# ALVI-Labs/frankenstein

Hardware: AMD Instinct MI355X
Metric: neural frames/sec (train fwd+bwd+AdamW, whole job) (higher is better)
Workload: dtype bf16; 1 GPU; brainformer-small (6L d=384 6x64 heads, N=6144 tokens) + 2-block perceiver, L1 head; fwd+bwd+clip+AdamW; per_gpu_batch=32, global_batch=32, frames_T=600, electrodes=256, parallelism=dp1, weights=random-init (seed 42)

## Files before the change

### frankenstein_amd/csrc/mlp_fused.hip

```cpp
#include "fk_common.h"

namespace {

#include "gemm_tile.h"

typedef __attribute__((address_space(3))) void lds_void_t;
typedef __attribute__((address_space(1))) const void glb_void_t;
extern __shared__ __attribute__((aligned(16))) char smem[];

struct MlpBwdArgs {
  const bf16_t* dy; const bf16_t* w2t; const bf16_t* h13; const bf16_t* w13t;
  bf16_t* dh13; bf16_t* dx;
  int64_t lddy, ldw2t, ldh, ldw13t, lddh, lddx;
  int M, H;
};

constexpr int MF_D = 384, MF_NW = 4, MF_TOK = MF_NW * 32;
constexpr int MF_KT = MF_D / 64;
constexpr int MF_NT = MF_D / 32;
constexpr int MF_W2 = MF_KT * 32 * ROW_BYTES;
constexpr int MF_W13 = MF_D * ROW_BYTES;
constexpr int MF_SLOT = MF_W2 + MF_W13;
constexpr int MF_HREG = 32 * ROW_BYTES;
constexpr int MF_LDS = 2 * MF_SLOT + MF_NW * MF_HREG;
constexpr int MF_P2 = MF_W2 / 1024 / MF_NW;
constexpr int MF_P13 = MF_W13 / 1024 / MF_NW;
constexpr int MF_ROWP = MF_D * 2 + 16;
static_assert(MF_LDS <= 160 * 1024 && MF_TOK * MF_ROWP <= MF_LDS, "LDS of a CU");
static_assert(MF_SLOT % (1024 * MF_NW) == 0, "whole pieces per wave");

template <bool FAST_SIGMOID> FK_DEV float mf_sigmoid(float x) {
  if constexpr (FAST_SIGMOID) return __builtin_amdgcn_rcpf(1.0f + __expf(-x));
  else return 1.0f / (1.0f + __expf(-x));
}

FK_DEV void mf_dma(const void* base, unsigned voff, unsigned dst) {
  asm volatile("s_mov_b32 m0, %2\n\ts_nop 0\n\tglobal_load_lds_dwordx4 %0, %1" ::"v"(voff), "s"(base), "s"(dst) : "memory");
}
FK_DEV void wait_all_barrier() { asm volatile("s_waitcnt vmcnt(0)\n\ts_barrier" ::: "memory"); }

struct LaneIds {
  int lane, li, lh, wave, row8, ch;
  FK_DEV LaneIds() {
    const int tid = threadIdx.x;
    lane = tid & 63, li = lane & 31, lh = lane >> 5;
    wave = __builtin_amdgcn_readfirstlane(tid >> 6);
    row8 = lane >> 3, ch = lane & 7;
  }
};
FK_DEV int swz_col(int r, int ch) { return (ch ^ ((r >> 1) & 7)) << 3; }
FK_DEV unsigned row_byte_off(int row, int64_t ld, int col) { return (unsigned)(((int64_t)row * ld + col) * 2); }

FK_DEV void load_token_frags(Frag<bf16_t> (&f)[MF_D / 16], const bf16_t* base, int row, int64_t ld, int lh) {
  const bf16_t* src = base + (int64_t)row * ld + 8 * lh;
#pragma unroll
  for (int t = 0; t < MF_D / 16; ++t) frag_load_contig<bf16_t>(f[t], src + 16 * t);
}
template <int N> FK_DEV void zero_acc(f32x16 (&a)[N]) {
#pragma unroll
  for (int t = 0; t < N; ++t)
#pragma unroll
    for (int r = 0; r < 16; ++r) a[t][r] = 0.0f;
}

template <int N> FK_DEV void row_segments(bf16_t* (&dst)[N], bool (&ok)[N], bf16_t* base, int64_t ld, int row0, int step, int M, int col) {
#pragma unroll
  for (int j = 0; j < N; ++j) {
    const int mr = row0 + j * step;
    ok[j] = mr < M;
    dst[j] = base + (int64_t)(ok[j] ? mr : M - 1) * ld + col;
  }
}
FK_DEV void read_tile_rows(bf16x8 (&rb)[4], const char* tile, const LaneIds& L) {
#pragma unroll
  for (int j = 0; j < 4; ++j) rb[j] = *reinterpret_cast<const bf16x8*>(tile + nt_off(j * 8 + L.row8, L.ch));
}
template <int N, bool NT> FK_DEV void store_rows(bf16_t* const (&dst)[N], const bool (&ok)[N], bool wave_full, int col, const bf16x8 (&v)[N]) {
  if (wave_full) {
#pragma unroll
    for (int j = 0; j < N; ++j) fk_st<NT>(reinterpret_cast<bf16x8*>(dst[j] + col), v[j]);
  } else {
#pragma unroll
    for (int j = 0; j < N; ++j)
      if (ok[j]) fk_st<NT>(reinterpret_cast<bf16x8*>(dst[j] + col), v[j]);
  }
}

struct BwdRing {
  const MlpBwdArgs& p;
  const LaneIds& L;
  unsigned lds0, off2[MF_P2], off13[MF_P13];
  FK_DEV BwdRing(const MlpBwdArgs& p_, const LaneIds& L_) : p(p_), L(L_), lds0((unsigned)(uintptr_t)(lds_void_t*)smem) {
#pragma unroll
    for (int j = 0; j < MF_P2; ++j) {
      const int q = L.wave * MF_P2 + j, s6 = q >> 2, r = (q & 3) * 8 + L.row8;
      off2[j] = (unsigned)((r * (int)p.ldw2t + s6 * 64 + swz_col(r, L.ch)) * 2);
    }
#pragma unroll
    for (int j = 0; j < MF_P13; ++j) {
      const int r = (L.wave * MF_P13 + j) * 8 + L.row8;
      off13[j] = (unsigned)((r * (int)p.ldw13t + swz_col(r, L.ch)) * 2);
    }
  }
  template <typename B> static FK_DEV B w2_at(B base, int slot) { return base + slot * MF_W2; }
  template <typename B> static FK_DEV B w13_at(B base, int slot) { return base + 2 * MF_W2 + slot * MF_W13; }
  template <typename B> FK_DEV B tile_at(B base) const { return base + 2 * MF_SLOT + L.wave * MF_HREG; }
  FK_DEV const char* w2img(int slot) const { return w2_at(smem, slot); }
  FK_DEV const char* w13img(int slot) const { return w13_at(smem, slot); }
  FK_DEV char* tile() const { return tile_at(smem); }
  FK_DEV unsigned tile_lds() const { return __builtin_amdgcn_readfirstlane(tile_at(lds0)); }
  FK_DEV const bf16_t* w2_src(int c) const { return p.w2t + (int64_t)c * 32 * p.ldw2t; }
  FK_DEV const bf16_t* w13_src(int c) const { return p.w13t + (int64_t)c * 64; }
  FK_DEV const bf16_t* h_src(int c) const { return p.h13 + (int64_t)c * 64; }
  FK_DEV unsigned w2_dst(int slot) const { return __builtin_amdgcn_readfirstlane(w2_at(lds0, slot) + L.wave * (MF_W2 / MF_NW)); }
  FK_DEV unsigned w13_dst(int slot) const { return __builtin_amdgcn_readfirstlane(w13_at(lds0, slot) + L.wave * (MF_W13 / MF_NW)); }
  FK_DEV void dma_w2(int c, int slot, int j) const { mf_dma(w2_src(c), off2[j], w2_dst(slot) + j * 1024); }
  FK_DEV void dma_w13(int c, int slot, int j) const { mf_dma(w13_src(c), off13[j], w13_dst(slot) + j * 1024); }
  FK_DEV unsigned h_off(int j, int row) const { return row_byte_off(row, p.ldh, swz_col(j * 8 + L.row8, L.ch)); }
  FK_DEV void dma_h(int c, int j, unsigned hoff, unsigned tile_dst) const { mf_dma(h_src(c), hoff, tile_dst + j * 1024); }
  FK_DEV void issue_w2(int c, int slot) const {
#pragma unroll
    for (int j = 0; j < MF_P2; ++j) dma_w2(c, slot, j);
  }
  FK_DEV void issue_w13(int c, int slot) const {
#pragma unroll
    for (int j = 0; j < MF_P13; ++j) dma_w13(c, slot, j);
  }
  FK_DEV void issue_h(int c, const unsigned (&hoff)[4], unsigned tile_dst) const {
#pragma unroll
    for (int j = 0; j < 4; ++j) dma_h(c, j, hoff[j], tile_dst);
  }
};

template <typename F>
FK_DEV void first_product(f32x16& dg, Frag<bf16_t> (&fa)[2][4], const char* w2img, const Frag<bf16_t> (&dyf)[MF_D / 16], const LaneIds& L, const F& behind) {
#pragma unroll
  for (int r = 0; r < 16; ++r) dg[r] = 0.0f;
#pragma unroll
  for (int s = 0; s < 4; ++s) nt_frag<bf16_t>(fa[0][s], w2img, L.li, s, L.lh);
#pragma unroll
  for (int s6 = 0; s6 < MF_KT; ++s6) {
    if (s6 + 1 < MF_KT) {
#pragma unroll
      for (int s = 0; s < 4; ++s) nt_frag<bf16_t>(fa[(s6 + 1) & 1][s], w2img + (s6 + 1) * 32 * ROW_BYTES, L.li, s, L.lh);
    }
#pragma unroll
    for (int s = 0; s < 4; ++s) mma32<bf16_t>(dg, fa[s6 & 1][s], dyf[s6 * 4 + s]);
    behind(s6);
    __builtin_amdgcn_sched_group_barrier(0x100, 4, 0);
    __builtin_amdgcn_sched_group_barrier(0x008, 4, 0);
    __builtin_amdgcn_sched_barrier(0);
  }
}

FK_DEV bf16x8 dswiglu_piece(const bf16x8& hv, const f32x16& dg, int s) {
  bf16x8 o;
#pragma unroll
  for (int e = 0; e < 4; ++e) {
    const float a1 = (float)hv[e], a3 = (float)hv[4 + e], g = dg[4 * s + e];
    const float sg = mf_sigmoid<true>(a1), ds = g * sg;
    o[e] = (bf16_t)(ds * a3 * (1.0f + a1 * (1.0f - sg)));
    o[4 + e] = (bf16_t)(ds * a1);
  }
  return o;
}

template <typename F>
FK_DEV void second_product(f32x16 (&dx)[MF_NT], Frag<bf16_t> (&fa)[2][4], const char* w13img, const Frag<bf16_t> (&bf)[4], const LaneIds& L, const F& behind) {
#pragma unroll
  for (int s = 0; s < 4; ++s) nt_frag<bf16_t>(fa[0][s], w13img, L.li, s, L.lh);
#pragma unroll
  for (int t = 0; t < MF_NT; ++t) {
    if (t + 1 < MF_NT) {
#pragma unroll
      for (int s = 0; s < 4; ++s) nt_frag<bf16_t>(fa[(t + 1) & 1][s], w13img, 32 * (t + 1) + L.li, s, L.lh);
    }
#pragma unroll
    for (int s = 0; s < 4; ++s) mma32<bf16_t>(dx[t], fa[t & 1][s], bf[s]);
    behind(t);
    __builtin_amdgcn_sched_group_barrier(0x100, 4, 0);
    __builtin_amdgcn_sched_group_barrier(0x008, 4, 0);
    __builtin_amdgcn_sched_barrier(0);
  }
}

FK_DEV void store_dx(const MlpBwdArgs& p, const f32x16 (&dx)[MF_NT], const LaneIds& L, int m0w, int row_end) {
  char* stg = smem + L.wave * 32 * MF_ROWP;
#pragma unroll
  for (int t = 0; t < MF_NT; ++t)
#pragma unroll
    for (int g = 0; g < 4; ++g) {
      bf16x4 v;
#pragma unroll
      for (int e = 0; e < 4; ++e) v[e] = (bf16_t)dx[t][4 * g + e];
      *reinterpret_cast<bf16x4*>(stg + L.li * MF_ROWP + (32 * t + 8 * g + 4 * L.lh) * 2) = v;
    }
  asm volatile("s_waitcnt lgkmcnt(0)" ::: "memory");
  if (L.lane < MF_D / 8) {
    for (int r = 0; r < 32; ++r) {
      if (m0w + r >= row_end) break;
      const bf16x8 v = *reinterpret_cast<const bf16x8*>(stg + r * MF_ROWP + L.lane * 16);
      fk_st<true>(reinterpret_cast<bf16x8*>(p.dx + (int64_t)(m0w + r) * p.lddx + L.lane * 8), v);
    }
  }
}

#ifdef MF_STAMP
__device__ unsigned long long mf_stamp_acc[16];
#define MF_ST_DECL unsigned long long st_acc[10] = {0, 0, 0, 0, 0, 0, 0, 0, 0, 0}; unsigned long long st_t = __builtin_amdgcn_s_memtime(); const unsigned long long st_t0 = st_t;
#define MF_ST(i) { const unsigned long long t_ = __builtin_amdgcn_s_memtime(); st_acc[i] += t_ - st_t; st_t = t_; }
#define MF_ST_FLUSH(lane) if ((lane) == 0) { for (int i_ = 0; i_ < 10; ++i_) atomicAdd(&mf_stamp_acc[i_], st_acc[i_]); atomicAdd(&mf_stamp_acc[15], __builtin_amdgcn_s_memtime() - st_t0); }
#else
#define MF_ST_DECL
#define MF_ST(i)
#define MF_ST_FLUSH(lane)
#endif

__global__ __launch_bounds__(MF_NW * 64, 1) void mlp_bwd_fused_kernel(MlpBwdArgs p) {
  using T = bf16_t;
  const LaneIds L;
  const BwdRing ring(p, L);
  const int m0w = blockIdx.x * MF_TOK + L.wave * 32, m = m0w + L.li;
  const int mc = m < p.M ? m : p.M - 1;
  const bool wave_full = m0w + 32 <= p.M;
  const int nchunks = p.H / 32, last = nchunks - 1;
  char* hreg = ring.tile();
  const unsigned hreg_lds = ring.tile_lds();
  T* hdst[4];
  bool hrow_ok[4];
  row_segments(hdst, hrow_ok, p.dh13, p.lddh, m0w + L.row8, 8, p.M, L.ch << 3);
  unsigned hoff[4];
#pragma unroll
  for (int j = 0; j < 4; ++j) hoff[j] = ring.h_off(j, hrow_ok[j] ? m0w + j * 8 + L.row8 : p.M - 1);

  ring.issue_w2(0, 0);
  ring.issue_w13(0, 0);
  ring.issue_w2(last < 1 ? last : 1, 1);
  ring.issue_h(0, hoff, hreg_lds);
  Frag<T> dyf[MF_D / 16];
  load_token_frags(dyf, p.dy, mc, p.lddy, L.lh);
  f32x16 dx[MF_NT];
  zero_acc(dx);
  wait_all_barrier();

  for (int c = 0; c < nchunks; ++c) {
    if (c > 0) asm volatile("s_waitcnt vmcnt(26)\n\ts_barrier" ::: "memory");
    const int cn1 = c + 1 < nchunks ? c + 1 : last, cn2 = c + 2 < nchunks ? c + 2 : last;
    f32x16 dg;
    Frag<T> fa[2][4];
    first_product(dg, fa, ring.w2img(c & 1), dyf, L, [&](int s6) __attribute__((always_inline)) {
      ring.dma_w13(cn1, (c + 1) & 1, 2 * s6);
      ring.dma_w13(cn1, (c + 1) & 1, 2 * s6 + 1);
    });
    asm volatile("s_waitcnt vmcnt(12)" ::: "memory");
    Frag<T> bf[4];
#pragma unroll
    for (int s = 0; s < 4; ++s) {
      bf[s].v = dswiglu_piece(*reinterpret_cast<const bf16x8*>(hreg + nt_off(L.li, 2 * s + L.lh)), dg, s);
      *reinterpret_cast<bf16x8*>(hreg + nt_off(L.li, 2 * s + L.lh)) = bf[s].v;
    }
    bf16x8 rb[4];
    read_tile_rows(rb, hreg, L);
    asm volatile("s_waitcnt vmcnt(22)\n\ts_barrier" ::: "memory");
    store_rows<4, true>(hdst, hrow_ok, wave_full, c * 64, rb);
    second_product(dx, fa, ring.w13img(c & 1), bf, L, [&](int t) __attribute__((always_inline)) {
      if (t < MF_P2) ring.dma_w2(cn2, c & 1, t);
      else if (t < MF_P2 + 4) ring.dma_h(cn1, t - MF_P2, hoff[t - MF_P2], hreg_lds);
    });
  }
  wait_all_barrier();
  store_dx(p, dx, L, m0w, p.M);
}


typedef unsigned u32x16 __attribute__((ext_vector_type(16)));
typedef unsigned u32x4v __attribute__((ext_vector_type(4)));
#ifndef FK_MLPB_INC
#define FK_MLPB_INC "mlp_bwd_asm.inc"
#endif
#include FK_MLPB_INC

__global__ __launch_bounds__(MF_NW * 64, 1) void mlp_bwd_fused_asm_kernel(MlpBwdArgs p) {
  MF_ST_DECL
  using T = bf16_t;
  const LaneIds L;
  const BwdRing ring(p, L);
  const int m0w = blockIdx.x * MF_TOK + L.wave * 32;
  const int nchunks = p.H / 32, last = nchunks - 1;
  auto cl = [&](int k) { return k < last ? k : last; };
  char* hreg = ring.tile();
  const unsigned hreg_lds = ring.tile_lds();
  u32x16 adr, ofs;
  unsigned ax[4], hoff[4];
#pragma unroll
  for (int s = 0; s < 4; ++s) {
    ax[s] = (unsigned)nt_off(L.li, 2 * s + L.lh);
    adr[4 + s] = hreg_lds + ax[s];
    adr[8 + s] = hreg_lds + (unsigned)nt_off(s * 8 + L.row8, L.ch);
  }
#pragma unroll
  for (int j = 0; j < MF_P2; ++j) ofs[j] = ring.off2[j];
#pragma unroll
  for (int j = 0; j < 4; ++j) {
    hoff[j] = ring.h_off(j, m0w + j * 8 + L.row8);
    ofs[6 + j] = hoff[j];
    ofs[10 + j] = row_byte_off(m0w + j * 8 + L.row8, p.lddh, L.ch << 3);
  }
  ofs[14] = 0;
  ofs[15] = 0;

  ring.issue_w2(0, 0);
  ring.issue_w13(0, 0);
  ring.issue_w2(cl(1), 1);
  ring.issue_h(0, hoff, hreg_lds);
  Frag<T> dyf[MF_D / 16];
  load_token_frags(dyf, p.dy, m0w + L.li, p.lddy, L.lh);
  f32x16 dx[MF_NT];
  zero_acc(dx);
  MF_ST(4)
  wait_all_barrier();
  MF_ST(5)
  Frag<T> fa[2][4];
  f32x16 dg;
  u32x16 fa0, bfc, bfn, hvv;
  first_product(dg, fa, ring.w2img(0), dyf, L, [](int) {});
  {
    bf16x8 rb[4];
#pragma unroll
    for (int s = 0; s < 4; ++s) {
      const bf16x8 o = dswiglu_piece(*reinterpret_cast<const bf16x8*>(hreg + nt_off(L.li, 2 * s + L.lh)), dg, s);
      *reinterpret_cast<bf16x8*>(hreg + nt_off(L.li, 2 * s + L.lh)) = o;
      const u32x4v w = __builtin_bit_cast(u32x4v, o);
#pragma unroll
      for (int k = 0; k < 4; ++k) bfc[4 * s + k] = w[k];
    }
    read_tile_rows(rb, hreg, L);
#pragma unroll
    for (int j = 0; j < 4; ++j)
      fk_st<true>(reinterpret_cast<bf16x8*>(p.dh13 + (int64_t)(m0w + j * 8 + L.row8) * p.lddh + (L.ch << 3)), rb[j]);
  }
  asm volatile("s_waitcnt lgkmcnt(0)\n\ts_barrier" ::: "memory");
  ring.issue_w2(cl(2), 0);
  ring.issue_h(cl(1), hoff, hreg_lds);
#pragma unroll
  for (int s = 0; s < 4; ++s) {
    const u32x4v w = *reinterpret_cast<const u32x4v*>(ring.w2img(1) + ax[s]);
#pragma unroll
    for (int k = 0; k < 4; ++k) fa0[4 * s + k] = w[k];
  }

  MF_ST(0)
  for (int c = 0; c < last; ++c) {
    const char* w2img = ring.w2img((c + 1) & 1);
    const char* w13img = ring.w13img(c & 1);
#pragma unroll
    for (int r = 0; r < 16; ++r) dg[r] = 0.0f;
#pragma unroll
    for (int s = 0; s < 4; ++s) {
      const u32x4v w = {fa0[4 * s], fa0[4 * s + 1], fa0[4 * s + 2], fa0[4 * s + 3]};
      fa[0][s].v = __builtin_bit_cast(bf16x8, w);
    }
#pragma unroll
    for (int s6 = 0; s6 < MF_KT; ++s6) {
      if (s6 + 1 < MF_KT) {
#pragma unroll
        for (int s = 0; s < 4; ++s) nt_frag<T>(fa[(s6 + 1) & 1][s], w2img + (s6 + 1) * 32 * ROW_BYTES, L.li, s, L.lh);
      } else {
        __builtin_amdgcn_sched_barrier(0);
        MF_ST(1)
        asm volatile("s_waitcnt vmcnt(10) lgkmcnt(0)\n\ts_barrier" ::: "memory");
        MF_ST(2)
#pragma unroll
        for (int s = 0; s < 4; ++s) {
          const u32x4v w = *reinterpret_cast<const u32x4v*>(w13img + ax[s]);
          const u32x4v h = *reinterpret_cast<const u32x4v*>(hreg + ax[s]);
#pragma unroll
          for (int k = 0; k < 4; ++k) { fa0[4 * s + k] = w[k]; hvv[4 * s + k] = h[k]; }
        }
      }
#pragma unroll
      for (int s = 0; s < 4; ++s) mma32<T>(dg, fa[s6 & 1][s], dyf[s6 * 4 + s]);
      ring.dma_w13(cl(c + 1), (c + 1) & 1, 2 * s6);
      ring.dma_w13(cl(c + 1), (c + 1) & 1, 2 * s6 + 1);
      if (s6 + 1 < MF_KT) __builtin_amdgcn_sched_group_barrier(0x100, 4, 0);
      else __builtin_amdgcn_sched_group_barrier(0x100, 8, 0);
      __builtin_amdgcn_sched_group_barrier(0x008, 4, 0);
      __builtin_amdgcn_sched_barrier(0);
    }
    MF_ST(3)
    const unsigned w13a = ring.w13_at(ring.lds0, c & 1), w2a = ring.w2_at(ring.lds0, c & 1);
#pragma unroll
    for (int s = 0; s < 4; ++s) {
      adr[s] = w13a + ax[s];
      adr[12 + s] = w2a + ax[s];
    }
    mlpb_step_asm(dx, dg, fa0, bfc, bfn, hvv, adr, ofs, ring.w2_src(cl(c + 3)), ring.h_src(cl(c + 2)), p.dh13 + (int64_t)(c + 1) * 64,
                  ring.w2_dst((c + 1) & 1), hreg_lds);
    bfc = bfn;
    MF_ST(6)
  }
  asm volatile("s_waitcnt vmcnt(0) lgkmcnt(0)\n\ts_barrier" ::: "memory");
  MF_ST(7)
  {
    Frag<T> bf[4];
#pragma unroll
    for (int s = 0; s < 4; ++s) {
      const u32x4v w = {bfc[4 * s], bfc[4 * s + 1], bfc[4 * s + 2], bfc[4 * s + 3]};
      bf[s].v = __builtin_bit_cast(bf16x8, w);
    }
    second_product(dx, fa, ring.w13img(last & 1), bf, L, [](int) {});
  }
  MF_ST(8)
  asm volatile("s_waitcnt lgkmcnt(0)\n\ts_barrier" ::: "memory");
  store_dx(p, dx, L, m0w, m0w + 32);
  MF_ST(9)
  MF_ST_FLUSH(L.lane)
}


struct MlpUpArgs {
  const bf16_t* x; const bf16_t* w13; bf16_t* h13; bf16_t* g;
  int64_t ldx, ldw, ldh, ldg;
  int M, H;
};
constexpr int MU_NW = 8, MU_TOK = MU_NW * 32;
constexpr int MU_TILE = MF_KT * 32 * ROW_BYTES;
constexpr int MU_SLOT = 2 * MU_TILE;
constexpr int MU_HT = 32 * ROW_BYTES, MU_GT = 32 * 64;
constexpr int MU_LDS = 2 * MU_SLOT + MU_NW * (MU_HT + MU_GT);
static_assert(MU_LDS <= 160 * 1024, "LDS of a CU");
constexpr int MU_PIECES = MU_SLOT / 1024 / MU_NW;

struct FwdRing {
  const bf16_t* w;
  int64_t ldw;
  unsigned lds0, woff[MU_PIECES];
  int wave;
  template <typename RowMap> FK_DEV FwdRing(const bf16_t* w_, int64_t ldw_, const LaneIds& L, const RowMap& wrow) : w(w_), ldw(ldw_), lds0((unsigned)(uintptr_t)(lds_void_t*)smem), wave(L.wave) {
#pragma unroll
    for (int j = 0; j < MU_PIECES; ++j) {
      const int q = L.wave * MU_PIECES + j, tile = q / 24, s6 = (q % 24) >> 2, n = (q & 3) * 8 + L.row8;
      woff[j] = (unsigned)((wrow(tile, n) * (int)ldw + s6 * 64 + swz_col(n, L.ch)) * 2);
    }
  }
  FK_DEV void issue_w(int c, int slot) const {
    const void* gw = w + (int64_t)c * 64 * ldw;
    const unsigned d = __builtin_amdgcn_readfirstlane(lds0 + slot * MU_SLOT + wave * (MU_SLOT / MU_NW));
#pragma unroll
    for (int j = 0; j < MU_PIECES; ++j) mf_dma(gw, woff[j], d + j * 1024);
  }
};

__global__ __launch_bounds__(MU_NW * 64, 2) void mlp_up_fused_kernel(MlpUpArgs p) {
  using T = bf16_t;
  const int tid = threadIdx.x, lane = tid & 63, li = lane & 31, lh = lane >> 5;
  const int wave = __builtin_amdgcn_readfirstlane(tid >> 6);
  const int m0w = blockIdx.x * MU_TOK + wave * 32;
  const int m = m0w + li, mc = m < p.M ? m : p.M - 1;
  const bool wave_full = m0w + 32 <= p.M;
  const int nchunks = p.H / 32, last = nchunks - 1;
  const int row8 = lane >> 3, ch = lane & 7;
  const unsigned lds0 = (unsigned)(uintptr_t)(lds_void_t*)smem;

  unsigned woff[MU_PIECES];
#pragma unroll
  for (int j = 0; j < MU_PIECES; ++j) {
    const int q = wave * MU_PIECES + j, tile = q / 24, s6 = (q % 24) >> 2, n = (q & 3) * 8 + row8;
    const int wrow = 8 * (n >> 2) + (n & 3) + 4 * tile;
    woff[j] = (unsigned)((wrow * (int)p.ldw + s6 * 64 + swz_col(n, ch)) * 2);
  }
  auto issue_w = [&](int c, int slot) __attribute__((always_inline)) {
    const void* gw = p.w13 + (int64_t)c * 64 * p.ldw;
    const unsigned d0 = __builtin_amdgcn_readfirstlane(lds0 + slot * MU_SLOT + wave * (MU_SLOT / MU_NW));
#pragma unroll
    for (int j = 0; j < MU_PIECES; ++j) mf_dma(gw, woff[j], d0 + j * 1024);
  };
  char* htile = smem + 2 * MU_SLOT + wave * (MU_HT + MU_GT);
  char* gtile = htile + MU_HT;
  T* hdst[4];
  T* gdst[2];
  bool hok[4], gok[2];
#pragma unroll
  for (int j = 0; j < 4; ++j) {
    const int mr = m0w + j * 8 + row8;
    hok[j] = mr < p.M;
    hdst[j] = p.h13 + (int64_t)(hok[j] ? mr : p.M - 1) * p.ldh + (ch << 3);
  }
#pragma unroll
  for (int j = 0; j < 2; ++j) {
    const int mr = m0w + j * 16 + (lane >> 2);
    gok[j] = mr < p.M;
    gdst[j] = p.g + (int64_t)(gok[j] ? mr : p.M - 1) * p.ldg + ((lane & 3) << 3);
  }

  issue_w(0, 0);
  Frag<T> xf[MF_D / 16];
  const T* xrow = p.x + (int64_t)mc * p.ldx + 8 * lh;
#pragma unroll
  for (int t = 0; t < MF_D / 16; ++t) frag_load_contig<T>(xf[t], xrow + 16 * t);
  wait_all_barrier();

  bf16x8 rbh[4] = {}, rbg[2] = {};
  for (int c = 0; c < nchunks; ++c) {
    const char* t0 = smem + (c & 1) * MU_SLOT;
    const char* t1 = t0 + MU_TILE;
    if (c > 0) {
      if (wave_full) {
#pragma unroll
        for (int j = 0; j < 4; ++j) fk_st<true>(reinterpret_cast<bf16x8*>(hdst[j] + (c - 1) * 64), rbh[j]);
#pragma unroll
        for (int j = 0; j < 2; ++j) fk_st<true>(reinterpret_cast<bf16x8*>(gdst[j] + (c - 1) * 32), rbg[j]);
      } else {
#pragma unroll
        for (int j = 0; j < 4; ++j)
          if (hok[j]) fk_st<true>(reinterpret_cast<bf16x8*>(hdst[j] + (c - 1) * 64), rbh[j]);
#pragma unroll
        for (int j = 0; j < 2; ++j)
          if (gok[j]) fk_st<true>(reinterpret_cast<bf16x8*>(gdst[j] + (c - 1) * 32), rbg[j]);
      }
    }
    issue_w(c + 1 < nchunks ? c + 1 : last, (c + 1) & 1);
    f32x16 a1, a3;
#pragma unroll
    for (int r = 0; r < 16; ++r) { a1[r] = 0.0f; a3[r] = 0.0f; }
    Frag<T> f1[2][4], f3[2][4];
#pragma unroll
    for (int s = 0; s < 4; ++s) { nt_frag<T>(f1[0][s], t0, li, s, lh); nt_frag<T>(f3[0][s], t1, li, s, lh); }
#pragma unroll
    for (int s6 = 0; s6 < MF_KT; ++s6) {
      if (s6 + 1 < MF_KT) {
#pragma unroll
        for (int s = 0; s < 4; ++s) {
          nt_frag<T>(f1[(s6 + 1) & 1][s], t0 + (s6 + 1) * 32 * ROW_BYTES, li, s, lh);
          nt_frag<T>(f3[(s6 + 1) & 1][s], t1 + (s6 + 1) * 32 * ROW_BYTES, li, s, lh);
        }
      }
#pragma unroll
      for (int s = 0; s < 4; ++s) {
        mma32<T>(a1, f1[s6 & 1][s], xf[s6 * 4 + s]);
        mma32<T>(a3, f3[s6 & 1][s], xf[s6 * 4 + s]);
      }
      __builtin_amdgcn_sched_group_barrier(0x100, 8, 0);
      __builtin_amdgcn_sched_group_barrier(0x008, 8, 0);
      __builtin_amdgcn_sched_barrier(0);
    }
#pragma unroll
    for (int g4 = 0; g4 < 4; ++g4) {
      bf16x8 hp;
      bf16x4 gp;
#pragma unroll
      for (int i = 0; i < 4; ++i) {
        const float h1 = a1[4 * g4 + i], h3 = a3[4 * g4 + i];
        hp[i] = (T)h1;
        hp[4 + i] = (T)h3;
        gp[i] = (T)(h1 * mf_sigmoid<true>(h1) * h3);
      }
      const int q = 2 * g4 + lh;
      *reinterpret_cast<bf16x8*>(htile + nt_off(li, q)) = hp;
      *reinterpret_cast<bf16x4*>(gtile + li * 64 + ((((q >> 1) + li) & 3) << 4) + ((q & 1) << 3)) = gp;
    }
#pragma unroll
    for (int j = 0; j < 4; ++j) rbh[j] = *reinterpret_cast<const bf16x8*>(htile + nt_off(j * 8 + row8, ch));
#pragma unroll
    for (int j = 0; j < 2; ++j) {
      const int r = j * 16 + (lane >> 2);
      rbg[j] = *reinterpret_cast<const bf16x8*>(gtile + r * 64 + ((((lane & 3) + r) & 3) << 4));
    }
    wait_all_barrier();
  }
  if (wave_full) {
#pragma unroll
    for (int j = 0; j < 4; ++j) fk_st<true>(reinterpret_cast<bf16x8*>(hdst[j] + last * 64), rbh[j]);
#pragma unroll
    for (int j = 0; j < 2; ++j) fk_st<true>(reinterpret_cast<bf16x8*>(gdst[j] + last * 32), rbg[j]);
  } else {
#pragma unroll
    for (int j = 0; j < 4; ++j)
      if (hok[j]) fk_st<true>(reinterpret_cast<bf16x8*>(hdst[j] + last * 64), rbh[j]);
#pragma unroll
    for (int j = 0; j < 2; ++j)
      if (gok[j]) fk_st<true>(reinterpret_cast<bf16x8*>(gdst[j] + last * 32), rbg[j]);
  }
}


struct QkvArgs {
  const bf16_t* x; const bf16_t* w; bf16_t* out; const float* table;
  int64_t ldx, ldw, ldo, table_bs, q_off;
  int M, N, T, pos_off, rot_chunks, q_chunks;
};
constexpr int QK_LDS = 2 * MU_SLOT + MU_NW * MU_HT;
static_assert(QK_LDS <= 160 * 1024, "LDS of a CU");

__global__ __launch_bounds__(MU_NW * 64, 2) void qkv_rope_fused_kernel(QkvArgs p) {
  using T = bf16_t;
  const LaneIds L;
  const int lh = L.lh;
  const int m0w = blockIdx.x * MU_TOK + L.wave * 32;
  const int m = m0w + L.li, mc = m < p.M ? m : p.M - 1;
  const bool wave_full = m0w + 32 <= p.M;
  const int nchunks = p.N / 64, last = nchunks - 1;
  const FwdRing ring(p.w, p.ldw, L, [](int tile, int n) { return 32 * tile + n; });
  char* htile = smem + 2 * MU_SLOT + L.wave * MU_HT;
  T* odst[4];
  bool ook[4];
  row_segments(odst, ook, p.out, p.ldo, m0w + L.row8, 8, p.M, L.ch << 3);
  const float* trow = p.table + (int64_t)(mc / p.T) * p.table_bs + (int64_t)(p.pos_off + mc % p.T) * 64 + 4 * lh;

  ring.issue_w(0, 0);
  Frag<T> xf[MF_D / 16];
  load_token_frags(xf, p.x, mc, p.ldx, lh);
  wait_all_barrier();

  bf16x8 rb[4] = {};
  for (int c = 0; c < nchunks; ++c) {
    const char* t0 = smem + (c & 1) * MU_SLOT;
    const char* t1 = t0 + MU_TILE;
    if (c > 0) store_rows<4, true>(odst, ook, wave_full, (c - 1) * 64, rb);
    const bool rot = c < p.rot_chunks;
    f32x4 cs[8];
    if (rot) {
      const float* tq = trow + (c < p.q_chunks ? p.q_off : (int64_t)0);
      asm volatile("global_load_dwordx4 %0, %8, off\n\tglobal_load_dwordx4 %1, %8, off offset:32\n\t"
                   "global_load_dwordx4 %2, %8, off offset:64\n\tglobal_load_dwordx4 %3, %8, off offset:96\n\t"
                   "global_load_dwordx4 %4, %8, off offset:128\n\tglobal_load_dwordx4 %5, %8, off offset:160\n\t"
                   "global_load_dwordx4 %6, %8, off offset:192\n\tglobal_load_dwordx4 %7, %8, off offset:224"
                   : "=&v"(cs[0]), "=&v"(cs[1]), "=&v"(cs[2]), "=&v"(cs[3]), "=&v"(cs[4]), "=&v"(cs[5]), "=&v"(cs[6]), "=&v"(cs[7])
                   : "v"(tq) : "memory");
    }
    ring.issue_w(c + 1 < nchunks ? c + 1 : last, (c + 1) & 1);
    f32x16 acc[2];
#pragma unroll
    for (int r = 0; r < 16; ++r) { acc[0][r] = 0.0f; acc[1][r] = 0.0f; }
    Frag<T> f[2][4];
#pragma unroll
    for (int s = 0; s < 4; ++s) nt_frag<T>(f[0][s], t0, L.li, s, lh);
#pragma unroll
    for (int gq = 0; gq < 2 * MF_KT; ++gq) {
      if (gq + 1 < 2 * MF_KT) {
        const char* nx = ((gq + 1) & 1 ? t1 : t0) + ((gq + 1) >> 1) * 32 * ROW_BYTES;
#pragma unroll
        for (int s = 0; s < 4; ++s) nt_frag<T>(f[(gq + 1) & 1][s], nx, L.li, s, lh);
      }
#pragma unroll
      for (int s = 0; s < 4; ++s) mma32<T>(acc[gq & 1], f[gq & 1][s], xf[(gq >> 1) * 4 + s]);
      __builtin_amdgcn_sched_group_barrier(0x100, 4, 0);
      __builtin_amdgcn_sched_group_barrier(0x008, 4, 0);
      __builtin_amdgcn_sched_barrier(0);
    }
    if (rot)
      asm volatile("s_waitcnt vmcnt(6)" : "+v"(cs[0]), "+v"(cs[1]), "+v"(cs[2]), "+v"(cs[3]), "+v"(cs[4]), "+v"(cs[5]), "+v"(cs[6]), "+v"(cs[7])::"memory");
#pragma unroll
    for (int tl = 0; tl < 2; ++tl)
#pragma unroll
      for (int g4 = 0; g4 < 4; ++g4) {
        float v[4] = {acc[tl][4 * g4], acc[tl][4 * g4 + 1], acc[tl][4 * g4 + 2], acc[tl][4 * g4 + 3]};
        if (rot) {
          const f32x4 t = cs[4 * tl + g4];
#pragma unroll
          for (int j = 0; j < 2; ++j) {
            const float re = v[2 * j], im = v[2 * j + 1];
            v[2 * j] = __builtin_fmaf(re, t[2 * j], -(im * t[2 * j + 1]));
            v[2 * j + 1] = __builtin_fmaf(re, t[2 * j + 1], im * t[2 * j]);
          }
        }
        bf16x4 o;
#pragma unroll
        for (int e = 0; e < 4; ++e) o[e] = (T)v[e];
        *reinterpret_cast<bf16x4*>(htile + nt_off(L.li, 4 * tl + g4) + 8 * lh) = o;
      }
    read_tile_rows(rb, htile, L);
    wait_all_barrier();
  }
  store_rows<4, true>(odst, ook, wave_full, last * 64, rb);
}

}

static bool mu_grid_fills(int64_t M) {
  const int64_t wg = fk_cdiv(M, MU_TOK), rounds = fk_cdiv(wg, 256);
  return wg * 10 >= rounds * 256 * 7;
}
bool fk_qkv_rope_fused_ok(int64_t M, int64_t N, int64_t K, int64_t lda, int64_t ldb, int64_t ldc, bool has_bias, int64_t T, int64_t D, int64_t rot_cols,
                          int64_t q_cols, int dtype) {
  return dtype == FK_BF16 && K == MF_D && D == 64 && N > 0 && N < (1LL << 31) && N % 64 == 0 && rot_cols % 64 == 0 && q_cols % 64 == 0 && rot_cols <= N && !has_bias &&
         mu_grid_fills(M) && M < (1LL << 31) && T > 0 && M % T == 0 && lda % 8 == 0 && ldb % 8 == 0 && ldc % 8 == 0 && lda >= K && ldb >= K && ldc >= N &&
         64 * ldb * 2 < (1LL << 32);
}
int fk_qkv_rope_fused_launch(const void* A, int64_t lda, const void* W, int64_t ldb, void* C, int64_t ldc, int64_t M, int64_t N, const float* table,
                             int64_t table_bs, int64_t T, int64_t pos_off, int64_t rot_cols, int64_t q_cols, int64_t q_off, void* stream) {
  QkvArgs a{(const bf16_t*)A, (const bf16_t*)W, (bf16_t*)C, table, lda, ldb, ldc, table_bs, q_off, (int)M, (int)N, (int)T, (int)pos_off,
            (int)(rot_cols / 64), (int)(q_cols / 64)};
  fk_launch_lds<qkv_rope_fused_kernel>(dim3((unsigned)fk_cdiv(M, MU_TOK)), dim3(MU_NW * 64), QK_LDS, (hipStream_t)stream, a);
  FK_CHECK_LAUNCH("fk_gemm_nt_rope (token-on-the-lane kernel)");
  return FK_OK;
}

bool fk_mlp_up_fused_ok(int64_t M, int64_t H, int64_t K, int64_t lda, int64_t ldb, int64_t ldh, int64_t ldg, int dtype) {
  return dtype == FK_BF16 && K == MF_D && H > 0 && H < (1LL << 30) && H % 32 == 0 && mu_grid_fills(M) && M < (1LL << 31) && lda % 8 == 0 && ldb % 8 == 0 &&
         ldh % 8 == 0 && ldg % 8 == 0 && lda >= K && ldb >= K && ldh >= 2 * H && ldg >= H && 64 * ldb * 2 < (1LL << 32);
}
int fk_mlp_up_fused_launch(const void* A, int64_t lda, const void* W13, int64_t ldb, void* H13, int64_t ldh, void* G, int64_t ldg, int64_t M, int64_t H,
                           void* stream) {
  MlpUpArgs a{(const bf16_t*)A, (const bf16_t*)W13, (bf16_t*)H13, (bf16_t*)G, lda, ldb, ldh, ldg, (int)M, (int)H};
  fk_launch_lds<mlp_up_fused_kernel>(dim3((unsigned)fk_cdiv(M, MU_TOK)), dim3(MU_NW * 64), MU_LDS, (hipStream_t)stream, a);
  FK_CHECK_LAUNCH("fk_gemm_nt_swiglu (token-on-the-lane kernel)");
  return FK_OK;
}

#ifdef MF_STAMP
extern "C" int fk_debug_mf_stamps(unsigned long long* out, int reset) {
  hipDeviceSynchronize();
  hipMemcpyFromSymbol(out, HIP_SYMBOL(mf_stamp_acc), sizeof(unsigned long long) * 16);
  if (reset) { unsigned long long z[16] = {0}; hipMemcpyToSymbol(HIP_SYMBOL(mf_stamp_acc), z, sizeof(z)); }
  return 0;
}
#endif

extern "C" int fk_mlp_bwd_fused_route(int64_t M, int64_t lddh) {
  FK_CHECK_ARG(M > 0 && lddh > 0, "fk_mlp_bwd_fused_route: bad problem M=%lld lddh=%lld", (long long)M, (long long)lddh);
  return M % MF_TOK == 0 && M * lddh * 2 < (1LL << 32) ? FK_MLP_BWD_ASM : FK_MLP_BWD_HIPCC;
}

extern "C" int fk_mlp_bwd_fused(const void* dY, int64_t lddy, const void* W2T, int64_t ldw2t, const void* H13, int64_t ldh, const void* W13T,
                                int64_t ldw13t, void* dH13, int64_t lddh, void* dX, int64_t lddx, int64_t M, int64_t H, int64_t D, int dtype,
                                void* stream) {
  FK_CHECK_ARG(dtype == FK_BF16, "fk_mlp_bwd_fused: bf16 only (dtype %d)", dtype);
  FK_CHECK_ARG(D == MF_D, "fk_mlp_bwd_fused: model dimension %lld (built for %d)", (long long)D, MF_D);
  FK_CHECK_ARG(M > 0 && M < (1LL << 31) && H > 0 && H % 32 == 0 && H < (1 << 24), "fk_mlp_bwd_fused: bad shape M=%lld H=%lld", (long long)M, (long long)H);
  FK_CHECK_ARG(dY && W2T && H13 && W13T && dH13 && dX, "fk_mlp_bwd_fused: null pointer");
  FK_CHECK_ARG(lddy % 8 == 0 && ldw2t % 8 == 0 && ldh % 8 == 0 && ldw13t % 8 == 0 && lddh % 8 == 0 && lddx % 8 == 0 && lddy >= D && ldw2t >= D &&
                   ldh >= 2 * H && lddh >= 2 * H && ldw13t >= 2 * H && lddx >= D,
               "fk_mlp_bwd_fused: leading dimensions must be multiples of 8 elements and cover their rows");
  FK_CHECK_ARG(M * ldh * 2 < (1LL << 32) && (int64_t)D * ldw13t * 2 < (1LL << 32) && 32 * ldw2t * 2 < (1LL << 32),
               "fk_mlp_bwd_fused: the h13 block must be addressable with 32-bit byte offsets (M * ldh < 2^31 elements)");
  FK_CHECK_ARG((((uintptr_t)dY | (uintptr_t)W2T | (uintptr_t)H13 | (uintptr_t)W13T | (uintptr_t)dH13 | (uintptr_t)dX) & 15) == 0,
               "fk_mlp_bwd_fused: pointers must be 16-byte aligned");
  MlpBwdArgs a{(const bf16_t*)dY, (const bf16_t*)W2T, (const bf16_t*)H13, (const bf16_t*)W13T, (bf16_t*)dH13, (bf16_t*)dX,
               lddy, ldw2t, ldh, ldw13t, lddh, lddx, (int)M, (int)H};
  if (fk_mlp_bwd_fused_route(M, lddh) == FK_MLP_BWD_ASM)
    fk_launch_lds<mlp_bwd_fused_asm_kernel>(dim3((unsigned)(M / MF_TOK)), dim3(MF_NW * 64), MF_LDS, (hipStream_t)stream, a);
  else
    fk_launch_lds<mlp_bwd_fused_kernel>(dim3((unsigned)fk_cdiv(M, MF_TOK)), dim3(MF_NW * 64), MF_LDS, (hipStream_t)stream, a);
  FK_CHECK_LAUNCH("fk_mlp_bwd_fused");
  return FK_OK;
}
```

Before: 407,900 frames/s.

## Add software-pipelined MLP up-projection kernel overlapping epilogue with next chunk MMAs

```diff
diff --git a/frankenstein_amd/csrc/mlp_fused.hip b/frankenstein_amd/csrc/mlp_fused.hip
--- a/frankenstein_amd/csrc/mlp_fused.hip
+++ b/frankenstein_amd/csrc/mlp_fused.hip
@@ -418,6 +418,38 @@
 }
 
 
+#ifdef MU_NO_ARITH
+#define MU_GATE(x) 1.0f
+#else
+#define MU_GATE(x) mf_sigmoid<true>(x)
+#endif
+#if defined(MU_NO_STORE)
+#define MU_ST_H(...)
+#define MU_ST_G(...)
+#define MU_ROT_YOUNGER "0"
+#elif defined(MU_NO_H)
+#define MU_ST_H(...)
+#define MU_ST_G(...) fk_st<true>(__VA_ARGS__)
+#define MU_ROT_YOUNGER "2"
+#elif defined(MU_NO_G)
+#define MU_ST_H(...) fk_st<true>(__VA_ARGS__)
+#define MU_ST_G(...)
+#define MU_ROT_YOUNGER "4"
+#else
+#ifdef MU_PLAIN_STORE
+#define MU_ST_H(...) fk_st<false>(__VA_ARGS__)
+#define MU_ST_G(...) fk_st<false>(__VA_ARGS__)
+#else
+#define MU_ST_H(...) fk_st<true>(__VA_ARGS__)
+#define MU_ST_G(...) fk_st<true>(__VA_ARGS__)
+#endif
+#define MU_ROT_YOUNGER "6"
+#endif
+#ifdef MU_NO_BARRIER
+#define MU_ROT_BARRIER ""
+#else
+#define MU_ROT_BARRIER "s_barrier"
+#endif
 struct MlpUpArgs {
   const bf16_t* x; const bf16_t* w13; bf16_t* h13; bf16_t* g;
   int64_t ldx, ldw, ldh, ldg;
@@ -443,6 +475,8 @@
       woff[j] = (unsigned)((wrow(tile, n) * (int)ldw + s6 * 64 + swz_col(n, L.ch)) * 2);
     }
   }
+  FK_DEV const void* src(int c) const { return w + (int64_t)c * 64 * ldw; }
+  FK_DEV unsigned dst(int slot) const { return __builtin_amdgcn_readfirstlane(lds0 + slot * MU_SLOT + wave * (MU_SLOT / MU_NW)); }
   FK_DEV void issue_w(int c, int slot) const {
     const void* gw = w + (int64_t)c * 64 * ldw;
     const unsigned d = __builtin_amdgcn_readfirstlane(lds0 + slot * MU_SLOT + wave * (MU_SLOT / MU_NW));
@@ -504,6 +538,10 @@
   for (int c = 0; c < nchunks; ++c) {
     const char* t0 = smem + (c & 1) * MU_SLOT;
     const char* t1 = t0 + MU_TILE;
+#ifdef MU_COUNTED_WAIT
+    issue_w(c + 1 < nchunks ? c + 1 : last, (c + 1) & 1);
+#endif
+#ifndef MU_NO_STORE
     if (c > 0) {
       if (wave_full) {
 #pragma unroll
@@ -519,7 +557,10 @@
           if (gok[j]) fk_st<true>(reinterpret_cast<bf16x8*>(gdst[j] + (c - 1) * 32), rbg[j]);
       }
     }
+#endif
+#ifndef MU_COUNTED_WAIT
     issue_w(c + 1 < nchunks ? c + 1 : last, (c + 1) & 1);
+#endif
     f32x16 a1, a3;
 #pragma unroll
     for (int r = 0; r < 16; ++r) { a1[r] = 0.0f; a3[r] = 0.0f; }
@@ -553,7 +594,7 @@
         const float h1 = a1[4 * g4 + i], h3 = a3[4 * g4 + i];
         hp[i] = (T)h1;
         hp[4 + i] = (T)h3;
-        gp[i] = (T)(h1 * mf_sigmoid<true>(h1) * h3);
+        gp[i] = (T)(h1 * MU_GATE(h1) * h3);
       }
       const int q = 2 * g4 + lh;
       *reinterpret_cast<bf16x8*>(htile + nt_off(li, q)) = hp;
@@ -566,8 +607,13 @@
       const int r = j * 16 + (lane >> 2);
       rbg[j] = *reinterpret_cast<const bf16x8*>(gtile + r * 64 + ((((lane & 3) + r) & 3) << 4));
     }
+#ifdef MU_COUNTED_WAIT
+    if (c > 0 && wave_full) asm volatile("s_waitcnt vmcnt(6)\n\ts_barrier" ::: "memory");
+    else
+#endif
     wait_all_barrier();
   }
+#ifndef MU_NO_STORE
   if (wave_full) {
 #pragma unroll
     for (int j = 0; j < 4; ++j) fk_st<true>(reinterpret_cast<bf16x8*>(hdst[j] + last * 64), rbh[j]);
@@ -580,6 +626,145 @@
 #pragma unroll
     for (int j = 0; j < 2; ++j)
       if (gok[j]) fk_st<true>(reinterpret_cast<bf16x8*>(gdst[j] + last * 32), rbg[j]);
+  }
+#endif
+}
+
+
+template <bool B> struct BoolC { static constexpr bool value = B; };
+
+__global__ __launch_bounds__(MU_NW * 64, 2) void mlp_up_fused_rot_kernel(MlpUpArgs p) {
+  using T = bf16_t;
+  const LaneIds L;
+  const int li = L.li, lh = L.lh;
+  const int m0w = blockIdx.x * MU_TOK + L.wave * 32;
+  const int nchunks = p.H / 32, last = nchunks - 1;
+  const FwdRing ring(p.w13, p.ldw, L, [](int tile, int n) { return 8 * (n >> 2) + (n & 3) + 4 * tile; });
+  char* htile = smem + 2 * MU_SLOT + L.wave * (MU_HT + MU_GT);
+  char* gtile = htile + MU_HT;
+  T* hdst[4];
+  T* gdst[2];
+  bool hok[4], gok[2];
+  row_segments(hdst, hok, p.h13, p.ldh, m0w + L.row8, 8, p.M, L.ch << 3);
+  row_segments(gdst, gok, p.g, p.ldg, m0w + (L.lane >> 2), 16, p.M, (L.lane & 3) << 3);
+
+  ring.issue_w(0, 0);
+  Frag<T> xf[MF_D / 16];
+  load_token_frags(xf, p.x, m0w + li, p.ldx, lh);
+  wait_all_barrier();
+
+  auto step = [&](auto tail, int c, f32x16& a1, f32x16& a3, const f32x16& p1, const f32x16& p3) __attribute__((always_inline)) {
+    constexpr bool TAIL = decltype(tail)::value;
+    const char* t0 = smem + (c & 1) * MU_SLOT;
+    const char* t1 = t0 + MU_TILE;
+    const void* wsrc = ring.src(c + 1 < nchunks ? c + 1 : last);
+    const unsigned wdst = ring.dst((c + 1) & 1);
+#pragma unroll
+    for (int r = 0; r < 16; ++r) { a1[r] = 0.0f; a3[r] = 0.0f; }
+    Frag<T> f1[4], f3[4];
+    auto read_frags = [&](int k) __attribute__((always_inline)) {
+      nt_frag<T>(f1[k & 3], t0 + (k >> 2) * 32 * ROW_BYTES, li, k & 3, lh);
+      nt_frag<T>(f3[k & 3], t1 + (k >> 2) * 32 * ROW_BYTES, li, k & 3, lh);
+    };
+    read_frags(0);
+    read_frags(1);
+#ifdef MU_NO_FRAG
+    read_frags(2);
+    read_frags(3);
+#endif
+    float gv[4];
+    bf16x8 hp, rbh[4];
+    bf16x4 gp;
+    bf16x8 rbg[2];
+    const int hcol = (c - 1) * 64, gcol = (c - 1) * 32;
+#pragma unroll
+    for (int k = 0; k < 4 * MF_KT; ++k) {
+#ifndef MU_NO_FRAG
+      if (k + 2 < 4 * MF_KT) read_frags(k + 2);
+#endif
+      mma32<T>(a1, f1[k & 3], xf[k]);
+      mma32<T>(a3, f3[k & 3], xf[k]);
+#ifndef MU_NO_DMA
+      if (k >= 2 && k < 2 + 2 * MU_PIECES && !(k & 1)) mf_dma(wsrc, ring.woff[(k - 2) >> 1], wdst + ((k - 2) >> 1) * 1024);
+#endif
+      if constexpr (TAIL) {
+        if (k < 16) {
+          const int g4 = k >> 2, i = k & 3;
+          const float h1 = p1[4 * g4 + i], h3 = p3[4 * g4 + i];
+          gv[i] = h1 * MU_GATE(h1) * h3;
+          if (i & 1) {
+            hp[i - 1] = (T)p1[4 * g4 + i - 1];
+            hp[i] = (T)h1;
+            hp[4 + i - 1] = (T)p3[4 * g4 + i - 1];
+            hp[4 + i] = (T)h3;
+            gp[i - 1] = (T)gv[i - 1];
+            gp[i] = (T)gv[i];
+          }
+          if (i == 3) {
+            const int q = 2 * g4 + lh;
+            *reinterpret_cast<bf16x8*>(htile + nt_off(li, q)) = hp;
+            *reinterpret_cast<bf16x4*>(gtile + li * 64 + ((((q >> 1) + li) & 3) << 4) + ((q & 1) << 3)) = gp;
+          }
+        } else if (k == 16) {
+#pragma unroll
+          for (int j = 0; j < 4; ++j) rbh[j] = *reinterpret_cast<const bf16x8*>(htile + nt_off(j * 8 + L.row8, L.ch));
+        } else if (k == 17) {
+#pragma unroll
+          for (int j = 0; j < 2; ++j) {
+            const int r = j * 16 + (L.lane >> 2);
+            rbg[j] = *reinterpret_cast<const bf16x8*>(gtile + r * 64 + ((((L.lane & 3) + r) & 3) << 4));
+          }
+        }
+        if (k >= 18 && k < 22) MU_ST_H(reinterpret_cast<bf16x8*>(hdst[k - 18] + hcol), rbh[k - 18]);
+        if (k >= 22) MU_ST_G(reinterpret_cast<bf16x8*>(gdst[k - 22] + gcol), rbg[k - 22]);
+      }
+      __builtin_amdgcn_sched_group_barrier(0x100, 2, 0);
+      __builtin_amdgcn_sched_group_barrier(0x008, 1, 0);
+      __builtin_amdgcn_sched_group_barrier(0x002, 6, 0);
+      __builtin_amdgcn_sched_group_barrier(0x008, 1, 0);
+      __builtin_amdgcn_sched_barrier(0);
+    }
+    if constexpr (TAIL) asm volatile("s_waitcnt vmcnt(" MU_ROT_YOUNGER ")\n\t" MU_ROT_BARRIER ::: "memory");
+    else wait_all_barrier();
+  };
+  auto tail_alone = [&](int c, const f32x16& p1, const f32x16& p3) __attribute__((always_inline)) {
+#pragma unroll
+    for (int g4 = 0; g4 < 4; ++g4) {
+      bf16x8 hp;
+      bf16x4 gp;
+#pragma unroll
+      for (int i = 0; i < 4; ++i) {
+        const float h1 = p1[4 * g4 + i], h3 = p3[4 * g4 + i];
+        hp[i] = (T)h1;
+        hp[4 + i] = (T)h3;
+        gp[i] = (T)(h1 * MU_GATE(h1) * h3);
+      }
+      const int q = 2 * g4 + lh;
+      *reinterpret_cast<bf16x8*>(htile + nt_off(li, q)) = hp;
+      *reinterpret_cast<bf16x4*>(gtile + li * 64 + ((((q >> 1) + li) & 3) << 4) + ((q & 1) << 3)) = gp;
+    }
+#pragma unroll
+    for (int j = 0; j < 4; ++j)
+      fk_st<true>(reinterpret_cast<bf16x8*>(hdst[j] + c * 64), *reinterpret_cast<const bf16x8*>(htile + nt_off(j * 8 + L.row8, L.ch)));
+#pragma unroll
+    for (int j = 0; j < 2; ++j) {
+      const int r = j * 16 + (L.lane >> 2);
+      fk_st<true>(reinterpret_cast<bf16x8*>(gdst[j] + c * 32), *reinterpret_cast<const bf16x8*>(gtile + r * 64 + ((((L.lane & 3) + r) & 3) << 4)));
+    }
+  };
+
+  f32x16 a1A, a3A, a1B, a3B;
+  step(BoolC<false>{}, 0, a1A, a3A, a1A, a3A);
+  int c = 1;
+  for (; c + 1 < nchunks; c += 2) {
+    step(BoolC<true>{}, c, a1B, a3B, a1A, a3A);
+    step(BoolC<true>{}, c + 1, a1A, a3A, a1B, a3B);
+  }
+  if (c < nchunks) {
+    step(BoolC<true>{}, c, a1B, a3B, a1A, a3A);
+    tail_alone(c, a1B, a3B);
+  } else {
+    tail_alone(c - 1, a1A, a3A);
   }
 }
 
@@ -681,6 +866,10 @@
   const int64_t wg = fk_cdiv(M, MU_TOK), rounds = fk_cdiv(wg, 256);
   return wg * 10 >= rounds * 256 * 7;
 }
+static bool lane_rot_enabled() {
+  const char* e = getenv("FK_LANE_ROT");
+  return !(e && e[0] == '0' && e[1] == 0);
+}
 bool fk_qkv_rope_fused_ok(int64_t M, int64_t N, int64_t K, int64_t lda, int64_t ldb, int64_t ldc, bool has_bias, int64_t T, int64_t D, int64_t rot_cols,
                           int64_t q_cols, int dtype) {
   return dtype == FK_BF16 && K == MF_D && D == 64 && N > 0 && N < (1LL << 31) && N % 64 == 0 && rot_cols % 64 == 0 && q_cols % 64 == 0 && rot_cols <= N && !has_bias &&
@@ -703,7 +892,10 @@
 int fk_mlp_up_fused_launch(const void* A, int64_t lda, const void* W13, int64_t ldb, void* H13, int64_t ldh, void* G, int64_t ldg, int64_t M, int64_t H,
                            void* stream) {
   MlpUpArgs a{(const bf16_t*)A, (const bf16_t*)W13, (bf16_t*)H13, (bf16_t*)G, lda, ldb, ldh, ldg, (int)M, (int)H};
-  fk_launch_lds<mlp_up_fused_kernel>(dim3((unsigned)fk_cdiv(M, MU_TOK)), dim3(MU_NW * 64), MU_LDS, (hipStream_t)stream, a);
+  if (M % MU_TOK == 0 && lane_rot_enabled())
+    fk_launch_lds<mlp_up_fused_rot_kernel>(dim3((unsigned)(M / MU_TOK)), dim3(MU_NW * 64), MU_LDS, (hipStream_t)stream, a);
+  else
+    fk_launch_lds<mlp_up_fused_kernel>(dim3((unsigned)fk_cdiv(M, MU_TOK)), dim3(MU_NW * 64), MU_LDS, (hipStream_t)stream, a);
   FK_CHECK_LAUNCH("fk_gemm_nt_swiglu (token-on-the-lane kernel)");
   return FK_OK;
 }
```

After: 409,700 frames/s, median of 6. Within noise of the previous version (+0.4%).
